# vuyraj/Data-Compression-Implementing-GPU-Driven-Huffman-Encoding-in-Java

Hardware: AMD Instinct MI355X
Metric: encode+decode GB/s (input bytes) (higher is better)
Workload: dtype u8

## Files before the change

data-compression-implementing-gpu-driven-huffman-encoding-in-java_amd/csrc/k1_histogram.hip:

```cpp
#include "dcz_internal.h"

namespace dcz {

#ifndef DCZ_K1_COPIES
#define DCZ_K1_COPIES 16
#endif
#ifndef DCZ_K1_NT
#define DCZ_K1_NT 1
#endif
#ifndef DCZ_K1_COPY_NT
#define DCZ_K1_COPY_NT 1
#endif
#ifndef DCZ_K1_COPY_LATE
#define DCZ_K1_COPY_LATE 1
#endif
#ifndef DCZ_K1_WAVES
#define DCZ_K1_WAVES 4
#endif
#ifndef DCZ_K1_RUNS
#define DCZ_K1_RUNS 1
#endif
constexpr int K1_WAVES = DCZ_K1_WAVES;
constexpr int K1_COPIES = DCZ_K1_COPIES;
constexpr int K1_CSHIFT = (K1_COPIES == 32) ? 5 : (K1_COPIES == 16) ? 4 : 3;
// ... 8 lines not shown
template <int K>
__device__ __forceinline__ void hist_add_byte(uint32_t hcol_addr, uint32_t d) {
    typedef __attribute__((address_space(3))) uint32_t lds_u32;
    uint32_t t, addr, b, val;
    asm("v_bfe_u32 %0, %1, %2, 7" : "=v"(t) : "v"(d), "n"(8 * K));
    asm("v_lshl_add_u32 %0, %1, %2, %3" : "=v"(addr) : "v"(t), "n"(K1_CSHIFT + 2), "v"(hcol_addr));
    asm("v_bfe_u32 %0, %1, %2, 1" : "=v"(b) : "v"(d), "n"(8 * K + 7));
    asm("v_mad_u32_u24 %0, %1, %2, 1" : "=v"(val) : "v"(b), "s"(0xFFFFu));
    __hip_atomic_fetch_add((lds_u32*)(uintptr_t)addr, val, __ATOMIC_RELAXED, __HIP_MEMORY_SCOPE_WAVEFRONT);
}

__device__ __forceinline__ void hist_add_dword(uint32_t* h, uint32_t col, uint32_t d) {
    const uint32_t hcol_addr = (uint32_t)(uintptr_t)((__attribute__((address_space(3))) uint32_t*)(h + col));
    hist_add_byte<0>(hcol_addr, d);
    hist_add_byte<1>(hcol_addr, d);
    hist_add_byte<2>(hcol_addr, d);
    hist_add_byte<3>(hcol_addr, d);
}

__device__ __forceinline__ void hist_add_vec(uint32_t* h, uint32_t col, const uint4& v) {
    hist_add_dword(h, col, v.x);
    hist_add_dword(h, col, v.y);
    hist_add_dword(h, col, v.z);
    hist_add_dword(h, col, v.w);
}

__device__ __forceinline__ bool unit_is_run(const uint4& v) {
    return v.x == v.y && v.x == v.z && v.x == v.w && v.x == __builtin_amdgcn_alignbit(v.x, v.x, 8);
}
__device__ __forceinline__ void hist_add_vec_runs(uint32_t* h, uint32_t col, const uint4& v) {
    if (unit_is_run(v)) {
        const uint32_t byte = v.x & 0xFFu;
        const uint32_t idx = ((byte & 127u) << K1_CSHIFT) + col;
        const uint32_t val = ((byte >> 7) * 0xFFFFu + 1u) << 4;
        __hip_atomic_fetch_add(&h[idx], val, __ATOMIC_RELAXED, __HIP_MEMORY_SCOPE_WAVEFRONT);
    } else {
        hist_add_vec(h, col, v);
    }
}

template <bool COPY>
__global__ __launch_bounds__(K1_WAVES * 64) void k1_histogram(const uint8_t* __restrict__ in, size_t n,
                                                               size_t block_bytes, uint32_t spb, uint64_t nseg,
                                                               uint16_t* __restrict__ seg_hist,
                                                               uint8_t* __restrict__ copy_out) {
    __shared__ __attribute__((aligned(16))) uint32_t lds[K1_WAVES][K1_DW];
    const int w = (int)(threadIdx.x >> 6);
    const int lane = lane_id();
    const uint64_t seg = (uint64_t)blockIdx.x * K1_WAVES + (uint64_t)w;
    if (seg >= nseg) return;
    uint32_t* h = lds[w];
    const uint32_t col = (uint32_t)lane & (uint32_t)(K1_COPIES - 1);

    {
        uint4* h4 = reinterpret_cast<uint4*>(h);
        const uint4 z = make_uint4(0, 0, 0, 0);
#pragma unroll
        for (int i = 0; i < K1_DW / 4 / 64; i++) h4[i * 64 + lane] = z;
    }
    wave_lds_fence();

    const uint64_t b = seg / spb, j = seg % spb;
    const uint64_t bstart = b * (uint64_t)block_bytes;
    const uint64_t bend = (bstart + block_bytes < n) ? bstart + block_bytes : (uint64_t)n;
    const uint64_t s0 = bstart + j * (uint64_t)SEG;
    uint32_t len = 0;
    if (s0 < bend) len = (uint32_t)((bend - s0 < SEG) ? bend - s0 : SEG);
    const uint8_t* p = in + s0;

    uint32_t nhead = (uint32_t)((16u - ((uintptr_t)p & 15u)) & 15u);
    if (nhead > len) nhead = len;
    if ((uint32_t)lane < nhead) {
        const uint8_t v = p[lane];
        hist_add(h, col, v);
        if constexpr (COPY) copy_out[s0 + lane] = v;
    }
    const uint4* pv = reinterpret_cast<const uint4*>(p + nhead);
    u32x4* const cv = COPY ? reinterpret_cast<u32x4*>(copy_out + s0 + nhead) : nullptr;
    auto store4 = [&](uint32_t base, const uint4& d0, const uint4& d1, const uint4& d2, const uint4& d3) {
        if constexpr (COPY) {
            const uint32_t i0 = base + (uint32_t)lane;
            const u32x4 a = {d0.x, d0.y, d0.z, d0.w}, b2 = {d1.x, d1.y, d1.z, d1.w};
            const u32x4 c = {d2.x, d2.y, d2.z, d2.w}, e = {d3.x, d3.y, d3.z, d3.w};
#if DCZ_K1_COPY_NT
            __builtin_nontemporal_store(a, cv + i0);
            __builtin_nontemporal_store(b2, cv + i0 + 64);
            __builtin_nontemporal_store(c, cv + i0 + 128);
            __builtin_nontemporal_store(e, cv + i0 + 192);
#else
            cv[i0] = a;
            cv[i0 + 64] = b2;
            cv[i0 + 128] = c;
            cv[i0 + 192] = e;
#endif
        }
    };
    const uint32_t nvec = (len - nhead) >> 4;

    auto load4 = [&](uint32_t base, uint4& d0, uint4& d1, uint4& d2, uint4& d3) {
        const uint32_t i0 = base + (uint32_t)lane;
#if DCZ_K1_NT
        const u32x4* pn = reinterpret_cast<const u32x4*>(pv);
        const u32x4 n0 = __builtin_nontemporal_load(pn + i0), n1 = __builtin_nontemporal_load(pn + i0 + 64);
        const u32x4 n2 = __builtin_nontemporal_load(pn + i0 + 128), n3 = __builtin_nontemporal_load(pn + i0 + 192);
        d0 = make_uint4(n0.x, n0.y, n0.z, n0.w);
        d1 = make_uint4(n1.x, n1.y, n1.z, n1.w);
        d2 = make_uint4(n2.x, n2.y, n2.z, n2.w);
        d3 = make_uint4(n3.x, n3.y, n3.z, n3.w);
#else
        d0 = pv[i0];
        d1 = pv[i0 + 64];
        d2 = pv[i0 + 128];
        d3 = pv[i0 + 192];
#endif
    };
    const uint32_t nfull = nvec & ~255u;
    uint4 c0, c1, c2, c3;
    if (nfull) load4(0, c0, c1, c2, c3);
    for (uint32_t base = 0; base < nfull; base += 256) {
        uint4 n0 = c0, n1 = c1, n2 = c2, n3 = c3;
        if (base + 256 < nfull) load4(base + 256, n0, n1, n2, n3);
#if !DCZ_K1_COPY_LATE
        store4(base, c0, c1, c2, c3);
#endif
        if (DCZ_K1_RUNS && __builtin_popcountll(__builtin_amdgcn_ballot_w64(unit_is_run(c0))) >= 32) {
            hist_add_vec_runs(h, col, c0);
            hist_add_vec_runs(h, col, c1);
            hist_add_vec_runs(h, col, c2);
            hist_add_vec_runs(h, col, c3);
        } else {
            hist_add_vec(h, col, c0);
            hist_add_vec(h, col, c1);
            hist_add_vec(h, col, c2);
            hist_add_vec(h, col, c3);
        }
#if DCZ_K1_COPY_LATE
        store4(base, c0, c1, c2, c3);
#endif
        c0 = n0;
        c1 = n1;
        c2 = n2;
        c3 = n3;
    }
    for (uint32_t i = nfull + (uint32_t)lane; i < nvec; i += 64) {
        const uint4 v = pv[i];
        hist_add_vec(h, col, v);
        if constexpr (COPY) {
            const u32x4 a = {v.x, v.y, v.z, v.w};
            __builtin_nontemporal_store(a, cv + i);
        }
    }
    {
        const uint32_t done = nhead + (nvec << 4);
        const uint32_t ntail = len - done;
        if ((uint32_t)lane < ntail) {
            const uint8_t v = p[done + lane];
            hist_add(h, col, v);
            if constexpr (COPY) copy_out[s0 + done + lane] = v;
        }
    }
    wave_lds_fence();

    uint32_t acc0 = 0, acc1 = 0;
    const uint4* r0 = reinterpret_cast<const uint4*>(h + (uint32_t)lane * (uint32_t)K1_COPIES);
    const uint4* r1 = reinterpret_cast<const uint4*>(h + ((uint32_t)lane + 64u) * (uint32_t)K1_COPIES);
    constexpr int NQ = K1_COPIES / 4;
#pragma unroll
    for (int t = 0; t < NQ; t++) {
        const int q = (t + (lane >> 1)) & (NQ - 1);
        const uint4 a = r0[q];
        const uint4 c = r1[q];
// ... 44 lines not shown
```

data-compression-implementing-gpu-driven-huffman-encoding-in-java_amd/csrc/k4_dfa.hip:

```cpp
#include <cstdlib>
#include <utility>

#include "dcz_internal.h"

namespace dcz {

#ifndef DCZ_DFA_W
#define DCZ_DFA_W 256
#endif
#ifndef DCZ_DFA_OC
#define DCZ_DFA_OC 16384
#endif
#ifndef DCZ_DFA_HOIST
#define DCZ_DFA_HOIST 1
#endif
#define DFA_RJ_DECL uint32_t rfresh_ = 0
#define DFA_RJ(rj, ALWAYS)                                                     \
    if constexpr ((j & 7) == 0 && ((ALWAYS) || (j >> 3) >= HOIST_DW)) {        \
        rfresh_ = R[j >> 3];                                                   \
        asm volatile("" : "+v"(rfresh_));                                      \
    }                                                                          \
    const uint32_t rj = ((ALWAYS) || (j >> 3) >= HOIST_DW) ? rfresh_ : R[j >> 3]
#ifndef DCZ_DFA_HOIST_DW_SPLIT
#define DCZ_DFA_HOIST_DW_SPLIT 3
#endif
#ifndef DCZ_DFA_HOIST_DW_REC
#define DCZ_DFA_HOIST_DW_REC 0
#endif
#ifndef DCZ_DFA_HOIST_DW_COUNT
#define DCZ_DFA_HOIST_DW_COUNT 8
#endif
#ifndef DCZ_DFA_HOIST_DW_1024
#define DCZ_DFA_HOIST_DW_1024 5
#endif
#ifndef DCZ_DFA_X_FROM
#define DCZ_DFA_X_FROM 16
#endif
#ifndef DCZ_DFA_KATTR
#define DCZ_DFA_KATTR
#endif
#ifndef DCZ_DFA_ALLWALK
#define DCZ_DFA_ALLWALK 0
#endif
#ifndef DCZ_DFA_X6_BIT0
#define DCZ_DFA_X6_BIT0 64
#endif
#ifndef DCZ_DFA_X_FROM_SPARSE
#define DCZ_DFA_X_FROM_SPARSE 48
#endif
#ifndef DCZ_DFA_SPARSE_OC
#define DCZ_DFA_SPARSE_OC 16384
#endif
#ifndef DCZ_DFA_ABL
#define DCZ_DFA_ABL 0
#endif
#ifndef DCZ_DFA_DBG
#define DCZ_DFA_DBG 0
#endif
#ifndef DCZ_DFA_X6
#define DCZ_DFA_X6 1
#endif
#ifndef DCZ_DFA_RECORD
#define DCZ_DFA_RECORD 1
#endif
#ifndef DCZ_DFA_MINWAVES
#define DCZ_DFA_MINWAVES 4
#endif
#define DFA_OC_DECODE (DCZ_DFA_RECORD ? -1 : DCZ_DFA_OC)
#ifndef DCZ_K4_EXACT_AFTER
#define DCZ_K4_EXACT_AFTER 12
#endif
#ifndef DCZ_K4_CLS2_A
#define DCZ_K4_CLS2_A 4
#endif
#ifndef DCZ_K4_CLS2_B
#define DCZ_K4_CLS2_B 9
#endif

constexpr uint32_t DFA_ERR = 255;

#ifndef DCZ_DFA_SLOT_SMALL
#define DCZ_DFA_SLOT_SMALL 88
#endif
#ifndef DCZ_DFA_REC_AVG
#define DCZ_DFA_REC_AVG 60
#endif
constexpr int dfa_slot(int W) { return W > 512 ? 136 : DCZ_DFA_SLOT_SMALL; }
#ifndef DCZ_DFA_PCAP
#define DCZ_DFA_PCAP 12
#endif
constexpr int DFA_PCAP = DCZ_DFA_PCAP;
template <int W, int OC, int PL = 0>
struct DfaLds {
    static constexpr int CAP = (OC < 0) ? (16 + dfa_slot(W) * W - 512) : (OC + 512);
    static constexpr int TILE_BYTES = PL ? (OC + 64) : (CAP + 640);
    __attribute__((aligned(16))) uint32_t T[256 * 16];
    union {
        __attribute__((aligned(16))) uint32_t tile[TILE_BYTES / 4];
        struct {
            uint32_t node_p[256];
            uint32_t first[34], cnt[34], offs[34], nint[34], base[34];
            uint8_t node_l[256];
            uint8_t symtab[256], len8[256];
        };
    };
    uint16_t plist[PL ? W * (PL + 1) + 128 : 2];
    uint8_t exits[W];
    uint32_t wsum[W / 64];
    uint32_t flag[3];
    uint32_t maxlen, nstates, err_idx, cend_vote, zsym;
    int bad_table;
};

template <int W, class LdsT>
__device__ __forceinline__ uint32_t dfa_block_scan(uint32_t v, LdsT& L, uint32_t& total) {
    const uint32_t inc = wave_inclusive_scan_u32(v);
    __syncthreads();
    if ((threadIdx.x & 63u) == 63u) L.wsum[threadIdx.x >> 6] = inc;
    __syncthreads();
    uint32_t base = 0, tot = 0;
#pragma unroll
    for (int w = 0; w < W / 64; w++) {
        const uint32_t sv = L.wsum[w];
        if (w < (int)(threadIdx.x >> 6)) base += sv;
        tot += sv;
    }
    total = tot;
    return base + inc - v;
}

template <int Q>
__device__ __forceinline__ uint4 dfa_shift(const uint4& a, const uint4& b, uint32_t r) {
    const uint32_t d[8] = {a.x, a.y, a.z, a.w, b.x, b.y, b.z, b.w};
    return make_uint4(__builtin_amdgcn_alignbyte(d[Q + 1], d[Q], r), __builtin_amdgcn_alignbyte(d[Q + 2], d[Q + 1], r),
                      __builtin_amdgcn_alignbyte(d[Q + 3], d[Q + 2], r), __builtin_amdgcn_alignbyte(d[Q + 4], d[Q + 3], r));
}

#if DCZ_DFA_DBG
__device__ unsigned long long dfa_dbg[8];
#endif
#if DCZ_K4_PROF
__device__ unsigned long long dfa_prof[12];
#define DFA_T(i)                                  \
    do {                                          \
        const unsigned long long t_ = clock64();  \
        pacc[i] += t_ - plast;                    \
        plast = t_;                               \
    } while (0)
#else
#define DFA_T(i) do { } while (0)
#endif

template <int W, int OC, int MODE, bool SPARSE>
__global__ __launch_bounds__(W, W > 512 ? 1 : DCZ_DFA_MINWAVES) DCZ_DFA_KATTR void k4_dfa(
    const uint8_t* __restrict__ comp, const unsigned long long* __restrict__ d_comp_off,
    const uint32_t* __restrict__ d_comp_size, const uint32_t* __restrict__ d_orig_size, const uint8_t* __restrict__ d_len,
    size_t out_stride, uint8_t* __restrict__ out, int32_t* __restrict__ d_status, long long* __restrict__ d_errpos,
    uint8_t* __restrict__ d_cls, const SplitDesc* __restrict__ sdp) {
    using LdsT = DfaLds<W, OC, SPARSE ? DFA_PCAP : 0>;
    constexpr bool SPLIT = MODE == 1, COUNT = MODE == 2;
    constexpr bool RECORD = OC < 0;
    static_assert(!RECORD || (!SPARSE && !COUNT), "only the decoding passes of the dense automaton record");
    constexpr int HOIST_DW = !DCZ_DFA_HOIST ? 0 : SPLIT ? DCZ_DFA_HOIST_DW_SPLIT : W > 512 ? DCZ_DFA_HOIST_DW_1024 : COUNT ? DCZ_DFA_HOIST_DW_COUNT : DCZ_DFA_HOIST_DW_REC;
    __shared__ LdsT L;
    typedef __attribute__((address_space(3))) const uint32_t lds_cu32;
    typedef __attribute__((address_space(3))) uint32_t lds_u32;
    uint32_t b = blockIdx.x, reg = 0;
    const int tid = (int)threadIdx.x;
#if DCZ_K4_PROF
    unsigned long long pacc[12] = {0, 0, 0, 0, 0, 0, 0, 0, 0, 0, 0, 0};
    unsigned long long plast = clock64();
#endif
    if constexpr (SPLIT) {
        if (!split_region_of(sdp, blockIdx.x, b, reg)) return;
        if (d_cls[b] != 2 || reg >= sdp->nreg[b]) return;
    } else if constexpr (COUNT) {
        if (!split_region_of(sdp, blockIdx.x, b, reg)) return;
        if (d_cls[b] != 0) return;
    } else {
        if (d_cls[b] != 0) return;
    }
    const uint32_t orig_blk = d_orig_size[b];
    const unsigned long long coff = d_comp_off[b];
    const uint32_t csize = d_comp_size[b];
    if constexpr (COUNT) {
        const unsigned long long S = sdp->region_bytes;
        const unsigned long long nreg = ((((uintptr_t)comp + (uintptr_t)coff) & 15u) + csize + S - 1) / S;
        if (nreg < 2 || reg >= nreg || nreg > sdp->rmax) return;
    }
    const uint32_t orig = SPLIT ? sdp->count[(uint64_t)b * sdp->rmax + reg] : COUNT ? 0xFFFFFFFFu : orig_blk;
    if (SPLIT && orig == 0u) return;
    {
        const bool long_codes = (unsigned long long)csize * 16ull >= (unsigned long long)orig_blk * 13ull;
        const bool medium = (unsigned long long)orig_blk * (unsigned long long)DCZ_K4_CLS2_A <=
                            (unsigned long long)csize * (unsigned long long)DCZ_K4_CLS2_B;
        if constexpr (SPARSE) {
            static_assert(!SPLIT, "regions of sparse blocks are decoded by k4_decode.hip");
            const bool sparse = (unsigned long long)csize * 80ull < (unsigned long long)orig_blk * 13ull;
            if (long_codes || medium || !sparse) return;
        } else {
            if (long_codes || !medium) return;
        }
    }

    if (tid < 34) L.cnt[tid] = 0;
    if (tid == 0) {
        L.bad_table = 0;
        L.err_idx = 0xFFFFFFFFu;
    }
    __syncthreads();
    for (int sy = tid; sy < 256; sy += W) {
        const uint32_t l = d_len[(uint64_t)b * 256u + sy];
        L.len8[sy] = (uint8_t)l;
        if (l > 32) L.bad_table = 1;
        else if (l > 0) atomicAdd(&L.cnt[l], 1u);
    }
    __syncthreads();
    if (tid == 0) {
        uint32_t c = 0, o = 0, mx = 0;
// ... 107 lines not shown
                    if (l > 32u) {
                        err = true;
                        break;
                    }
                    const uint32_t rel = p - L.first[l];
                    if (rel < L.cnt[l]) {
                        l = 0;
                        p = 0;
                    } else if (rel - L.cnt[l] >= L.nint[l]) {
                        err = true;
                    }
                }
                if (!err) next = L.base[l] + (p - L.first[l] - L.cnt[l]);
            }
            x6[idx] = (uint8_t)next;
        }
    }
    const uint32_t t_addr = (uint32_t)(uintptr_t)((__attribute__((address_space(3))) uint32_t*)(&L.T[0]));
    const uint32_t tile_addr = (uint32_t)(uintptr_t)((__attribute__((address_space(3))) uint32_t*)(&L.tile[0]));

    uint8_t* const oblk = out + (uint64_t)b * out_stride + (SPLIT ? sdp->off[(uint64_t)b * sdp->rmax + reg] : 0u);
    uint32_t hskip = SPLIT ? (uint32_t)(((uintptr_t)oblk) & 15u) : 0u;
    uint8_t* const obase = oblk - hskip;
    const bool out_aligned = (((uintptr_t)obase) & 15u) == 0u;
    const uintptr_t pay = (uintptr_t)comp + (uintptr_t)coff;
    const uint32_t skew = (uint32_t)(pay & 15u);
    const uint8_t* const vbase = reinterpret_cast<const uint8_t*>(pay - skew);
    const unsigned long long vlo = skew, vhi = (unsigned long long)skew + csize;

    uint32_t produced = 0, gpos = 0, ocarry = hskip;
    uint32_t entry0 = 0;
    unsigned long long wbyte = 0;
    uint32_t nwin = 0xFFFFFFFFu;
    bool preroll = false;
    if constexpr (SPLIT) {
        wbyte = (unsigned long long)reg * sdp->region_bytes;
        entry0 = sdp->entry[(uint64_t)b * sdp->rmax + reg];
    }
    if constexpr (COUNT) {
        const unsigned long long S = sdp->region_bytes;
        nwin = (uint32_t)(S / ((unsigned long long)W * 32ull));
        wbyte = (unsigned long long)reg * S;
        if (reg > 0) {
            wbyte -= (unsigned long long)W * 32ull;
            nwin++;
            preroll = true;
        }
    }
    int status = DCZ_OK;
    long long errpos = 0;
    constexpr uint32_t AMASK = SPARSE ? 0x3FC0u : 0xFFC0u;
    uint8_t* const ob = reinterpret_cast<uint8_t*>(L.tile);

    uint4 pre[3];
    auto prefetch = [&](unsigned long long wb) {
        const unsigned long long v0 = (wb + 32ull * (unsigned long long)tid + skew) & ~15ull;
#pragma unroll
        for (int c = 0; c < 3; c++) pre[c] = load_chunk16(vbase, v0 + 16ull * c, vlo, vhi);
    };
    const uint32_t sk2 = (skew + (uint32_t)(wbyte & 15ull)) & 15u;
    const uint32_t sq = sk2 >> 2, sr = sk2 & 3u;
    if (orig > 0 && wbyte < csize) prefetch(wbyte);
    const uint32_t slot_addr = tile_addr + 16u + (uint32_t)dfa_slot(W) * (uint32_t)tid;
    __syncthreads();
    const bool rec_block = RECORD && (dfa_slot(W) - 8 >= 128 || (unsigned long long)orig_blk * 32ull <=
                                                               (unsigned long long)csize * (unsigned long long)DCZ_DFA_REC_AVG);
    auto zero_tile = [&](uint32_t from16) {
        for (uint32_t i = from16 + (uint32_t)tid; i < (uint32_t)(sizeof(L.tile) / 16u); i += W)
            reinterpret_cast<uint4*>(L.tile)[i] = make_uint4(0u, 0u, 0u, 0u);
        __syncthreads();
    };
    if (!rec_block) zero_tile(0u);
    typedef __attribute__((address_space(3))) uint16_t lds_u16;
    typedef __attribute__((address_space(3))) uint8_t lds_u8;
    const uint32_t pl_addr = (uint32_t)(uintptr_t)((__attribute__((address_space(3))) uint16_t*)(&L.plist[0])) +
                             2u * (uint32_t)(DFA_PCAP + 1) * (uint32_t)tid;
    DFA_T(0);

    uint32_t rentry = 0, wexit = 0;
    unsigned long long rcount = 0;
    bool unusable = false;
    while (COUNT ? nwin != 0u : produced < orig) {
#if DCZ_K4_PROF
        pacc[8]++;
#endif
        uint32_t R[8];
        {
            uint4 lo, hi;
            switch (sq) {
                case 0: lo = dfa_shift<0>(pre[0], pre[1], sr); hi = dfa_shift<0>(pre[1], pre[2], sr); break;
                case 1: lo = dfa_shift<1>(pre[0], pre[1], sr); hi = dfa_shift<1>(pre[1], pre[2], sr); break;
                case 2: lo = dfa_shift<2>(pre[0], pre[1], sr); hi = dfa_shift<2>(pre[1], pre[2], sr); break;
                default: lo = dfa_shift<3>(pre[0], pre[1], sr); hi = dfa_shift<3>(pre[1], pre[2], sr); break;
            }
            R[0] = bswap32(lo.x);
            R[1] = bswap32(lo.y);
            R[2] = bswap32(lo.z);
            R[3] = bswap32(lo.w);
            R[4] = bswap32(hi.x);
            R[5] = bswap32(hi.y);
            R[6] = bswap32(hi.z);
            R[7] = bswap32(hi.w);
        }
        DFA_T(1);
        const bool exhausted = wbyte + (unsigned long long)W * 32ull >= csize;
        const bool beyond = wbyte + 32ull * (unsigned long long)tid >= csize;
        const bool more_payload = !exhausted;
        if (more_payload) prefetch(wbyte + (unsigned long long)W * 32ull);

        uint32_t g = (tid == 0) ? entry0 : 0u;
        uint32_t x = 0, nsym = 0, pc = 0;
        bool pover = false;
        bool need = !beyond;
        uint32_t round = (DCZ_DFA_ABL & 4) ? 1u : 0u;
        while (true) {
            if (DCZ_DFA_ALLWALK || __builtin_amdgcn_ballot_w64(need) != 0ull) {
                uint32_t e = g << 6, n = 0;
                if (round == 0u && small) {
                    constexpr int X6_BIT0 = DCZ_DFA_X6_BIT0, X6_STEPS = (256 - X6_BIT0) / 6;
                    static_assert(X6_BIT0 + 6 * X6_STEPS == 256, "the six-bit walk ends on the subsequence's last bit");
                    uint32_t rq[8], st6 = 0;
#pragma unroll
                    for (int k = X6_BIT0 >> 5; k < 8; k++) {
                        rq[k] = R[k];
                        asm volatile("" : "+v"(rq[k]));
                    }
                    auto stepX6 = [&](auto ic) __attribute__((always_inline)) {
                        constexpr int pbit = X6_BIT0 + 6 * decltype(ic)::value, k = pbit >> 5, off = pbit & 31;
                        uint32_t v;
                        if constexpr (off <= 26) v = (rq[k] >> (26 - off)) & 63u;
                        else v = __builtin_amdgcn_alignbit(rq[k], rq[k < 7 ? k + 1 : 7], 58 - off) & 63u;
                        st6 = (uint32_t)*(const lds_u8*)(uintptr_t)(t_addr + 8192u + ((st6 << 6) | v));
                    };
                    [&]<int... Is>(std::integer_sequence<int, Is...>) {
                        (stepX6(std::integral_constant<int, Is>{}), ...);
                    }(std::make_integer_sequence<int, X6_STEPS>{});
                    e = st6 << 6;
                } else if (round == 0u) {
                    constexpr int XF = SPARSE ? DCZ_DFA_X_FROM_SPARSE : DCZ_DFA_X_FROM;
                    if (XF > 0) e = 0;
                    DFA_RJ_DECL;
                    auto stepX = [&](auto jc) __attribute__((always_inline)) {
                        constexpr int j = decltype(jc)::value;
                        constexpr int sh = 26 - 4 * (j & 7);
                        DFA_RJ(rj, false);
                        const uint32_t nib4 = sh >= 0 ? ((rj >> (sh >= 0 ? sh : 0)) & 0x3Cu) : ((rj << 2) & 0x3Cu);
                        e = *(lds_cu32*)(uintptr_t)(t_addr + ((e & AMASK) | nib4));
                    };
                    [&]<int... Js>(std::integer_sequence<int, Js...>) {
                        (stepX(std::integral_constant<int, XF + Js>{}), ...);
                    }(std::make_integer_sequence<int, 64 - XF>{});
                } else if constexpr (SPARSE) {
                    uint32_t pa = pl_addr;
                    DFA_RJ_DECL;
                    auto stepP = [&](auto jc) __attribute__((always_inline)) {
                        constexpr int j = decltype(jc)::value;
                        constexpr int sh = 26 - 4 * (j & 7);
                        DFA_RJ(rj, false);
                        const uint32_t nib4 = sh >= 0 ? ((rj >> (sh >= 0 ? sh : 0)) & 0x3Cu) : ((rj << 2) & 0x3Cu);
                        e = *(lds_cu32*)(uintptr_t)(t_addr + ((e & AMASK) | nib4));
                        const uint32_t oth = e & 0x18u;
                        const uint32_t tp = n + ((e >> 14) & 3u);
                        *(lds_u16*)(uintptr_t)pa = (uint16_t)(tp | ((e >> 8) & 0xFF00u));
                        if (__builtin_amdgcn_ballot_w64(oth == 0x10u) != 0ull) {
                            if (oth == 0x10u) {
                                *(lds_u16*)(uintptr_t)pa = (uint16_t)(n | ((e >> 8) & 0xFF00u));
                                *(lds_u16*)(uintptr_t)(pa + 2u) = (uint16_t)(tp | ((e >> 16) & 0xFF00u));
                            }
                        }
                        pa += oth >> 2;
                        n += e & 7u;
                    };
                    [&]<int... Js>(std::integer_sequence<int, Js...>) {
                        (stepP(std::integral_constant<int, Js>{}), ...);
                    }(std::make_integer_sequence<int, 64>{});
                    if (need) pc = (pa - pl_addr) >> 1;
                } else if (RECORD && rec_block) {
                    uint32_t ab = slot_addr, k8 = 0, alo = 0;
#if DCZ_DFA_DBG
                    uint32_t chk = 0;
#endif
                    DFA_RJ_DECL;
                    auto stepR = [&](auto jc) __attribute__((always_inline)) {
                        constexpr int j = 2 * decltype(jc)::value;
                        constexpr int sh0 = 26 - 4 * (j & 7), sh1 = 26 - 4 * ((j + 1) & 7);
                        DFA_RJ(rj, false);
                        const uint32_t nib0 = (rj >> sh0) & 0x3Cu;
                        const uint32_t nib1 = sh1 >= 0 ? ((rj >> (sh1 >= 0 ? sh1 : 0)) & 0x3Cu) : ((rj << 2) & 0x3Cu);
                        const uint32_t e0 = *(lds_cu32*)(uintptr_t)(t_addr + ((e & AMASK) | nib0));
                        e = *(lds_cu32*)(uintptr_t)(t_addr + ((e0 & AMASK) | nib1));
                        const uint32_t c0 = e0 & 0x18u;
                        const uint32_t w = ((e >> 16) << c0) | (e0 >> 16);
                        const unsigned long long v = (unsigned long long)w << k8;
#if DCZ_DFA_DBG
                        chk = __builtin_amdgcn_sad_u8(w, 0u, chk);
#endif
                        alo |= (uint32_t)v;
                        *(lds_u32*)(uintptr_t)ab = alo;
                        k8 += c0 + (e & 0x18u);
                        const bool full = k8 >= 32u;
                        alo = full ? (uint32_t)(v >> 32) : alo;
                        ab += full ? 4u : 0u;
                        k8 &= 31u;
                    };
                    [&]<int... Js>(std::integer_sequence<int, Js...>) {
                        (stepR(std::integral_constant<int, Js>{}), ...);
                    }(std::make_integer_sequence<int, 32>{});
                    *(lds_u32*)(uintptr_t)ab = alo;
                    n = (ab - slot_addr) + (k8 >> 3);
#if DCZ_DFA_DBG
                    *(lds_u32*)(uintptr_t)(slot_addr + (uint32_t)dfa_slot(W) - 4u) = (n & 0xFFu) | (chk << 8);
#endif
                } else {
                    DFA_RJ_DECL;
                    auto stepA = [&](auto jc) __attribute__((always_inline)) {
                        constexpr int j = decltype(jc)::value;
                        constexpr int sh = 26 - 4 * (j & 7);
                        DFA_RJ(rj, RECORD || SPARSE);
                        const uint32_t nib4 = sh >= 0 ? ((rj >> (sh >= 0 ? sh : 0)) & 0x3Cu) : ((rj << 2) & 0x3Cu);
                        e = *(lds_cu32*)(uintptr_t)(t_addr + ((e & AMASK) | nib4));
                        n += e & (SPARSE ? 7u : 3u);
                    };
                    [&]<int... Js>(std::integer_sequence<int, Js...>) {
                        (stepA(std::integral_constant<int, Js>{}), ...);
                    }(std::make_integer_sequence<int, 64>{});
                }
                if (need) {
                    x = (e >> 6) & 0xFFu;
                    nsym = n;
                    if constexpr (SPARSE) pover |= pc > (uint32_t)DFA_PCAP;
                    else if constexpr (RECORD) pover |= n > (uint32_t)dfa_slot(W) - 8u;
                }
            }
            DFA_T(2);
#if DCZ_K4_PROF
            pacc[9]++;
#endif
            L.exits[tid] = (uint8_t)x;
            if (tid == 0) L.flag[(round + 1u) % 3u] = 0;
            __syncthreads();
            DFA_T(3);
            if (round > 1u && L.flag[round % 3u] == 0u) break;
            if (DCZ_DFA_ABL & 16) break;
            const uint32_t ng = (tid == 0) ? entry0 : (uint32_t)L.exits[tid - 1];
            need = ((ng != g) || round == 0u) && !beyond;
            g = ng;
            if (__builtin_amdgcn_ballot_w64(need) != 0ull && (tid & 63) == 0) L.flag[(round + 1u) % 3u] = 1;
            round++;
            if constexpr (MODE == 0 && !SPARSE) {
                if (round == (uint32_t)DCZ_K4_EXACT_AFTER) {
                    if (tid == 0) d_cls[b] = 1;
                    return;
                }
            }
            if constexpr (COUNT) {
                if (round == (uint32_t)DCZ_K4_EXACT_AFTER) {
                    if (tid == 0) sdp->exit[(uint64_t)b * sdp->rmax + reg] = 0xFFFFFFFFu;
                    return;
                }
            }
        }

        const bool bad = !beyond && x == errst;
        uint32_t tw = 0;
        constexpr uint32_t SLOT_SYMS = RECORD ? (uint32_t)dfa_slot(W) - 8u : 0u;
// ... 295 lines not shown
                        alo = ahi;
                        ahi = 0;
                        k8 -= 32u;
                        ab += 4u;
                    }
                };
                [&]<int... Js>(std::integer_sequence<int, Js...>) {
                    (stepB(std::integral_constant<int, Js>{}), ...);
                }(std::make_integer_sequence<int, 32>{});
            }
            __syncthreads();
            if (k8 != 0u)
                __hip_atomic_fetch_or((lds_u32*)(uintptr_t)ab, alo, __ATOMIC_RELAXED, __HIP_MEMORY_SCOPE_WORKGROUP);
            DFA_T(5);
#if DCZ_K4_PROF
            pacc[10]++;
#endif
            __syncthreads();
            DFA_T(6);
            const uint32_t total = ocarry + cc;
            const bool last = !more && cend == lim;
            const uint32_t full = last ? total : (total & ~15u);
            uint8_t* const dst = obase + gpos;
            const uint32_t nunits = (full + 15u) >> 4;
            for (uint32_t u = (uint32_t)tid; u < nunits; u += W) {
                const uint32_t lo = u << 4;
                const uint32_t* src = &L.tile[lo >> 2];
                if (out_aligned && lo + 16u <= full && lo >= hskip) {
                    *reinterpret_cast<uint4*>(dst + lo) = make_uint4(src[0], src[1], src[2], src[3]);
                } else {
                    for (uint32_t i = lo > hskip ? lo : hskip; i < lo + 16u && i < full; i++) dst[i] = ob[i];
                }
                *reinterpret_cast<uint4*>(&L.tile[lo >> 2]) = make_uint4(0u, 0u, 0u, 0u);
            }
            const uint32_t tail = total - full;
            uint8_t tv = 0;
            if ((uint32_t)tid < tail) tv = ob[full + tid];
            __syncthreads();
            if (full > 0u) {
                if (tid < 4) L.tile[(full >> 2) + (uint32_t)tid] = 0u;
                if ((uint32_t)tid < tail) ob[tid] = tv;
            }
            gpos += full;
            ocarry = tail;
            if (full > 0u) hskip = 0;
            cbase = cend;
            DFA_T(7);
            if (cbase < lim) __syncthreads();
        }
        }
        }
        produced += lim;
        entry0 = next_entry;
        wbyte += (unsigned long long)W * 32ull;
        if (exhausted && produced < orig) {
            __syncthreads();
            if ((uint32_t)tid < ocarry && (uint32_t)tid >= hskip) obase[gpos + tid] = (uint8_t)(ob[tid] ^ (SPARSE ? L.zsym : 0u));
            const uint8_t z = L.zsym;
            uint32_t fs = z;
            if (tid == 0) {
                uint32_t st = wexit;
                while (st != 0u) {
                    const uint32_t e = L.T[st * 16u];
                    if ((e & (SPARSE ? 7u : 3u)) != 0u) {
                        fs = (e >> 16) & 0xFFu;
                        break;
                    }
                    st = (e >> 6) & 0xFFu;
                    if (st == errst) {
                        status = DCZ_E_BADSTREAM;
                        errpos = (long long)produced;
                        break;
                    }
                }
            }
            for (uint32_t i = produced + (uint32_t)tid; i < orig; i += W) oblk[i] = (i == produced) ? (uint8_t)fs : z;
            break;
        }
        __syncthreads();
    }

    if constexpr (COUNT) {
        if (tid == 0) {
            const uint64_t i = (uint64_t)b * sdp->rmax + reg;
            const bool bad = unusable || wexit == errst || rentry == errst;
            sdp->entry[i] = rentry;
            sdp->count[i] = (uint32_t)(rcount > 0xFFFFFFFFull ? 0xFFFFFFFFull : rcount);
            sdp->exit[i] = bad ? 0xFFFFFFFFu : wexit;
        }
        return;
    }
    if (tid == 0 && (!SPLIT || status != DCZ_OK)) {
        d_status[b] = status;
        if (d_errpos) d_errpos[b] = errpos + (SPLIT ? (long long)sdp->off[(uint64_t)b * sdp->rmax + reg] : 0ll);
    }
#if DCZ_K4_PROF
    if (tid == 0)
        for (int i = 0; i < 12; i++) atomicAdd(&dfa_prof[i], pacc[i]);
#endif
}

void launch_count_dfa(const uint8_t* d_comp, const uint64_t* d_comp_off, const uint32_t* d_comp_size,
                      const uint32_t* d_orig_size, const uint8_t* d_len, uint8_t* d_cls, const SplitDesc* d_sd, hipStream_t s) {
    hipLaunchKernelGGL((k4_dfa<DCZ_DFA_W, 0, 2, false>), dim3(SPLIT_GRID), dim3(DCZ_DFA_W), 0, s, d_comp,
                       reinterpret_cast<const unsigned long long*>(d_comp_off), d_comp_size, d_orig_size, d_len, (size_t)0,
                       (uint8_t*)nullptr, (int32_t*)nullptr, (long long*)nullptr, d_cls, d_sd);
// ... 55 lines not shown
```

data-compression-implementing-gpu-driven-huffman-encoding-in-java_amd/csrc/k4_fixed.hip:

```cpp
#include "dcz_internal.h"

namespace dcz {

#ifndef DCZ_FX_TILE
#define DCZ_FX_TILE 8192
#endif
constexpr uint32_t FX_TILE = DCZ_FX_TILE;
#ifndef DCZ_FX_T
#define DCZ_FX_T 512
#endif
constexpr int FX_T = DCZ_FX_T;
constexpr int FX_UPT = (int)(FX_TILE / 16u / (uint32_t)FX_T);
static_assert(FX_T >= 256 && FX_UPT * FX_T * 16 == (int)FX_TILE, "tile = threads x units x 16 bytes");

__global__ __launch_bounds__(256) void k4_classify(const uint8_t* __restrict__ d_len,
                                                   const unsigned long long* __restrict__ d_comp_off,
                                                   const uint32_t* __restrict__ d_comp_size,
                                                   const uint32_t* __restrict__ d_orig_size, unsigned long long comp_bytes,
                                                   unsigned long long out_stride, uint32_t K, uint8_t* __restrict__ cls,
                                                   int32_t* __restrict__ d_status, long long* __restrict__ d_errpos,
                                                   uint32_t* __restrict__ hint, uint32_t* __restrict__ hint_done,
                                                   uint32_t epoch) {
    const uint32_t b = blockIdx.x * 256u + threadIdx.x;
    if (b >= K) return;
// ... 28 lines not shown
    cls[b] = c;
    if ((c & 0xF0u) == 0x10u && hint) *hint = epoch;
}

template <int Q>
__device__ __forceinline__ uint4 shift_units(const uint4& a, const uint4& b, uint32_t r) {
    const uint32_t d[8] = {a.x, a.y, a.z, a.w, b.x, b.y, b.z, b.w};
    return make_uint4(__builtin_amdgcn_alignbyte(d[Q + 1], d[Q], r), __builtin_amdgcn_alignbyte(d[Q + 2], d[Q + 1], r),
                      __builtin_amdgcn_alignbyte(d[Q + 3], d[Q + 2], r), __builtin_amdgcn_alignbyte(d[Q + 4], d[Q + 3], r));
}

__device__ __forceinline__ void store_unit(uint8_t* dst, const uint4& v, uint32_t nvalid, bool aligned) {
    if (aligned && nvalid >= 16u) {
        *reinterpret_cast<uint4*>(dst) = v;
    } else {
        const uint32_t w[4] = {v.x, v.y, v.z, v.w};
#pragma unroll
        for (int i = 0; i < 16; i++)
            if ((uint32_t)i < nvalid) dst[i] = (uint8_t)(w[i >> 2] >> (8 * (i & 3)));
    }
}

template <int L>
__device__ __forceinline__ uint4 extract16(const uint32_t (&bw)[5], const uint8_t* symtab) {
    uint32_t o[4] = {0, 0, 0, 0};
#pragma unroll
    for (int j = 0; j < 16; j++) {
        constexpr uint32_t mask = (1u << L) - 1u;
        const int bit = j * L, idx = bit >> 5, s = bit & 31;
        uint32_t v;
        if (s + L <= 32) v = (bw[idx] >> (32 - s - L)) & mask;
        else v = (uint32_t)((((unsigned long long)bw[idx] << 32) | bw[idx + 1]) >> (64 - s - L)) & mask;
        o[j >> 2] |= (uint32_t)symtab[v] << (8 * (j & 3));
    }
    return make_uint4(o[0], o[1], o[2], o[3]);
}

struct FxLds {
    __attribute__((aligned(16))) uint32_t stage[(FX_TILE / 8 * 7 + 64) / 4];
    uint8_t symtab[256];
    uint32_t wcnt[FX_T / 64];
};

__device__ __forceinline__ void fixed_item(FxLds& S, uint32_t b, uint32_t tile, const uint8_t* __restrict__ comp,
                                           const unsigned long long* __restrict__ d_comp_off,
                                           const uint32_t* __restrict__ d_comp_size,
                                           const uint32_t* __restrict__ d_orig_size, const uint8_t* __restrict__ d_len,
                                           unsigned long long out_stride, uint8_t* __restrict__ out,
                                           const uint8_t* __restrict__ cls) {
    uint32_t* const stage = S.stage;
    uint8_t* const symtab = S.symtab;
    uint32_t* const wcnt = S.wcnt;
    const uint32_t c = cls[b];
    if ((c & 0xF0u) != 0x10u) return;
    const uint32_t L = c & 15u;
    const int tid = (int)threadIdx.x;
    const uint32_t orig = d_orig_size[b];
    const unsigned long long t0 = (unsigned long long)tile * FX_TILE;
    if (t0 >= orig) return;
    const uint32_t nout = (orig - t0 < FX_TILE) ? (uint32_t)(orig - t0) : FX_TILE;
    const uintptr_t pay = (uintptr_t)comp + (uintptr_t)d_comp_off[b];
    const uint32_t skew = (uint32_t)(pay & 15u);
    const uint8_t* const vbase = reinterpret_cast<const uint8_t*>(pay - skew);
    const unsigned long long vlo = skew, vhi = (unsigned long long)skew + d_comp_size[b];
    uint8_t* const dst0 = out + (unsigned long long)b * out_stride + t0;
    const bool dst_al = (((uintptr_t)dst0) & 15u) == 0u;
    if (L == 8u) {
        if (skew == 0u && dst_al && nout == FX_TILE && t0 + FX_TILE <= vhi) {
            const u32x4* s4 = reinterpret_cast<const u32x4*>(vbase + t0) + tid;
            u32x4* d4 = reinterpret_cast<u32x4*>(dst0) + tid;
            u32x4 v[FX_UPT];
#pragma unroll
            for (int k = 0; k < FX_UPT; k++) v[k] = __builtin_nontemporal_load(s4 + FX_T * k);
#pragma unroll
            for (int k = 0; k < FX_UPT; k++) __builtin_nontemporal_store(v[k], d4 + FX_T * k);
            return;
        }
        uint4 v[FX_UPT];
        const uint32_t q = skew >> 2, r = skew & 3u;
#pragma unroll
        for (int k = 0; k < FX_UPT; k++) {
            const uint32_t o = ((uint32_t)tid + (uint32_t)FX_T * k) * 16u;
            v[k] = make_uint4(0, 0, 0, 0);
            if (o < nout) {
                const uint4 a = load_chunk16(vbase, t0 + o, vlo, vhi);
                if (skew == 0u) {
                    v[k] = a;
                } else {
                    const uint4 e = load_chunk16(vbase, t0 + o + 16u, vlo, vhi);
                    v[k] = (q == 0u) ? shift_units<0>(a, e, r) : (q == 1u) ? shift_units<1>(a, e, r)
                           : (q == 2u) ? shift_units<2>(a, e, r) : shift_units<3>(a, e, r);
                }
            }
        }
#pragma unroll
        for (int k = 0; k < FX_UPT; k++) {
            const uint32_t o = ((uint32_t)tid + (uint32_t)FX_T * k) * 16u;
            if (o < nout) store_unit(dst0 + o, v[k], nout - o, dst_al);
        }
        return;
    }
    {
        const bool present = tid < 256 && d_len[(uint64_t)b * 256u + (tid & 255)] != 0;
        const unsigned long long m = __builtin_amdgcn_ballot_w64(present);
        if (tid < 256 && (tid & 63) == 0) wcnt[tid >> 6] = (uint32_t)__builtin_popcountll(m);
        __syncthreads();
        uint32_t rank = (uint32_t)__builtin_popcountll(m & ((1ull << (tid & 63)) - 1ull));
        for (int w = 0; w < ((tid & 255) >> 6); w++) rank += wcnt[w];
        if (present) symtab[rank] = (uint8_t)tid;
    }
    const unsigned long long vin = (t0 >> 3) * L;
    const uint32_t nin = (nout * L + 7u) >> 3;
    const uint32_t nchunks = (skew + nin + 15u) >> 4;
    for (uint32_t ch = (uint32_t)tid; ch < nchunks; ch += FX_T)
        reinterpret_cast<uint4*>(stage)[ch] = load_chunk16(vbase, vin + 16ull * ch, vlo, vhi);
    __syncthreads();
#pragma unroll 1
// ... 111 lines not shown
```

Measured before the change: 1413.

## Overlap next-window DFA entry walk with current decode, defer histogram zeroing

The DFA decode kernel now computes the next window's starting state (the six-bit or nibble walk) while the current window's record/sparse walk is running, interleaving the independent LDS lookups to hide latency. The next payload is unpacked mid-walk, and the separate round-0 walk is skipped on later windows. The histogram kernel issues its first global loads before zeroing LDS and adding head bytes, and the fixed-length decoder hoists its metadata loads above the early return. This raises register pressure and code size and adds tail-masking logic for the pipelined unpack.

```diff
diff --git a/data-compression-implementing-gpu-driven-huffman-encoding-in-java_amd/csrc/k1_histogram.hip b/data-compression-implementing-gpu-driven-huffman-encoding-in-java_amd/csrc/k1_histogram.hip
--- a/data-compression-implementing-gpu-driven-huffman-encoding-in-java_amd/csrc/k1_histogram.hip
+++ b/data-compression-implementing-gpu-driven-huffman-encoding-in-java_amd/csrc/k1_histogram.hip
@@ -84,14 +84,6 @@
     uint32_t* h = lds[w];
     const uint32_t col = (uint32_t)lane & (uint32_t)(K1_COPIES - 1);
 
-    {
-        uint4* h4 = reinterpret_cast<uint4*>(h);
-        const uint4 z = make_uint4(0, 0, 0, 0);
-#pragma unroll
-        for (int i = 0; i < K1_DW / 4 / 64; i++) h4[i * 64 + lane] = z;
-    }
-    wave_lds_fence();
-
     const uint64_t b = seg / spb, j = seg % spb;
     const uint64_t bstart = b * (uint64_t)block_bytes;
     const uint64_t bend = (bstart + block_bytes < n) ? bstart + block_bytes : (uint64_t)n;
@@ -102,10 +94,10 @@
 
     uint32_t nhead = (uint32_t)((16u - ((uintptr_t)p & 15u)) & 15u);
     if (nhead > len) nhead = len;
+    uint8_t headv = 0;
     if ((uint32_t)lane < nhead) {
-        const uint8_t v = p[lane];
-        hist_add(h, col, v);
-        if constexpr (COPY) copy_out[s0 + lane] = v;
+        headv = p[lane];
+        if constexpr (COPY) copy_out[s0 + lane] = headv;
     }
     const uint4* pv = reinterpret_cast<const uint4*>(p + nhead);
     u32x4* const cv = COPY ? reinterpret_cast<u32x4*>(copy_out + s0 + nhead) : nullptr;
@@ -149,6 +141,14 @@
     const uint32_t nfull = nvec & ~255u;
     uint4 c0, c1, c2, c3;
     if (nfull) load4(0, c0, c1, c2, c3);
+    {
+        uint4* h4 = reinterpret_cast<uint4*>(h);
+        const uint4 z = make_uint4(0, 0, 0, 0);
+#pragma unroll
+        for (int i = 0; i < K1_DW / 4 / 64; i++) h4[i * 64 + lane] = z;
+    }
+    wave_lds_fence();
+    if ((uint32_t)lane < nhead) hist_add(h, col, headv);
     for (uint32_t base = 0; base < nfull; base += 256) {
         uint4 n0 = c0, n1 = c1, n2 = c2, n3 = c3;
         if (base + 256 < nfull) load4(base + 256, n0, n1, n2, n3);
diff --git a/data-compression-implementing-gpu-driven-huffman-encoding-in-java_amd/csrc/k4_dfa.hip b/data-compression-implementing-gpu-driven-huffman-encoding-in-java_amd/csrc/k4_dfa.hip
--- a/data-compression-implementing-gpu-driven-huffman-encoding-in-java_amd/csrc/k4_dfa.hip
+++ b/data-compression-implementing-gpu-driven-huffman-encoding-in-java_amd/csrc/k4_dfa.hip
@@ -48,6 +48,12 @@
 #ifndef DCZ_DFA_X_FROM_SPARSE
 #define DCZ_DFA_X_FROM_SPARSE 48
 #endif
+#ifndef DCZ_DFA_PIPE
+#define DCZ_DFA_PIPE 1
+#endif
+#ifndef DCZ_DFA_PIPE_1024
+#define DCZ_DFA_PIPE_1024 0
+#endif
 #ifndef DCZ_DFA_SPARSE_OC
 #define DCZ_DFA_SPARSE_OC 16384
 #endif
@@ -78,6 +84,15 @@
 #endif
 
 constexpr uint32_t DFA_ERR = 255;
+
+#ifndef DCZ_DFA_PIPE_LAG
+#define DCZ_DFA_PIPE_LAG 8
+#endif
+constexpr int dfa_x6_at(int i, int steps) {
+    constexpr int lag = DCZ_DFA_PIPE_LAG;
+    const int a = i < lag ? 0 : i < 2 * lag ? 2 * (i - lag) : i;
+    return a < steps ? a : steps;
+}
 
 #ifndef DCZ_DFA_SLOT_SMALL
 #define DCZ_DFA_SLOT_SMALL 88
@@ -165,6 +180,8 @@
     __shared__ LdsT L;
     typedef __attribute__((address_space(3))) const uint32_t lds_cu32;
     typedef __attribute__((address_space(3))) uint32_t lds_u32;
+    typedef __attribute__((address_space(3))) uint16_t lds_u16;
+    typedef __attribute__((address_space(3))) uint8_t lds_u8;
     uint32_t b = blockIdx.x, reg = 0;
     const int tid = (int)threadIdx.x;
 #if DCZ_K4_PROF
@@ -378,14 +395,78 @@
     constexpr uint32_t AMASK = SPARSE ? 0x3FC0u : 0xFFC0u;
     uint8_t* const ob = reinterpret_cast<uint8_t*>(L.tile);
 
+    typedef uint32_t u32x4 __attribute__((ext_vector_type(4)));
+    typedef __attribute__((address_space(1))) const u32x4 glb_cu4;
     uint4 pre[3];
     auto prefetch = [&](unsigned long long wb) {
         const unsigned long long v0 = (wb + 32ull * (unsigned long long)tid + skew) & ~15ull;
 #pragma unroll
-        for (int c = 0; c < 3; c++) pre[c] = load_chunk16(vbase, v0 + 16ull * c, vlo, vhi);
+        for (int c = 0; c < 3; c++) {
+            const unsigned long long vb = v0 + 16ull * c;
+            pre[c] = make_uint4(0u, 0u, 0u, 0u);
+            if (vb + 16ull > vlo && vb < vhi) {
+                const u32x4 t = *(glb_cu4*)(uintptr_t)(vbase + vb);
+                pre[c] = make_uint4(t.x, t.y, t.z, t.w);
+            }
+        }
     };
     const uint32_t sk2 = (skew + (uint32_t)(wbyte & 15ull)) & 15u;
     const uint32_t sq = sk2 >> 2, sr = sk2 & 3u;
+    auto unpack = [&](uint32_t (&d)[8], unsigned long long wb, uint32_t sr) __attribute__((always_inline)) {
+        uint4 lo, hi;
+        switch (sq) {
+            case 0: lo = dfa_shift<0>(pre[0], pre[1], sr); hi = dfa_shift<0>(pre[1], pre[2], sr); break;
+            case 1: lo = dfa_shift<1>(pre[0], pre[1], sr); hi = dfa_shift<1>(pre[1], pre[2], sr); break;
+            case 2: lo = dfa_shift<2>(pre[0], pre[1], sr); hi = dfa_shift<2>(pre[1], pre[2], sr); break;
+            default: lo = dfa_shift<3>(pre[0], pre[1], sr); hi = dfa_shift<3>(pre[1], pre[2], sr); break;
+        }
+        d[0] = bswap32(lo.x);
+        d[1] = bswap32(lo.y);
+        d[2] = bswap32(lo.z);
+        d[3] = bswap32(lo.w);
+        d[4] = bswap32(hi.x);
+        d[5] = bswap32(hi.y);
+        d[6] = bswap32(hi.z);
+        d[7] = bswap32(hi.w);
+        if (wb + (unsigned long long)W * 32ull > csize) {
+            const unsigned long long pb = wb + 32ull * (unsigned long long)tid;
+            const uint32_t nv = pb >= csize ? 0u : csize - pb >= 32ull ? 32u : (uint32_t)(csize - pb);
+#pragma unroll
+            for (int k = 0; k < 8; k++) {
+                const uint32_t vk = nv > 4u * k ? (nv - 4u * k < 4u ? nv - 4u * k : 4u) : 0u;
+                d[k] &= (uint32_t)(0xFFFFFFFF00000000ull >> (8u * vk));
+            }
+        }
+    };
+    auto unpack_next = [&](uint32_t (&d)[8], int from, unsigned long long wb) __attribute__((always_inline)) {
+        uint32_t srq = sr;
+        asm volatile("" : "+s"(srq));
+        unpack(d, wb, srq);
+#pragma unroll
+        for (int k = 0; k < 8; k++)
+            if (k >= from) asm volatile("" : "+v"(d[k]));
+    };
+    constexpr int X6_BIT0 = DCZ_DFA_X6_BIT0, X6_STEPS = (256 - X6_BIT0) / 6;
+    static_assert(X6_BIT0 + 6 * X6_STEPS == 256, "the six-bit walk ends on the subsequence's last bit");
+    auto x6step = [&](const uint32_t (&q)[8], uint32_t& st, auto ic) __attribute__((always_inline)) {
+        constexpr int pbit = X6_BIT0 + 6 * decltype(ic)::value, k = pbit >> 5, off = pbit & 31;
+        uint32_t v;
+        if constexpr (off <= 26) v = (q[k] >> (26 - off)) & 63u;
+        else v = __builtin_amdgcn_alignbit(q[k], q[k < 7 ? k + 1 : 7], 58 - off) & 63u;
+        st = (uint32_t)*(const lds_u8*)(uintptr_t)(t_addr + 8192u + ((st << 6) | v));
+    };
+    constexpr int XF = SPARSE ? DCZ_DFA_X_FROM_SPARSE : DCZ_DFA_X_FROM;
+    auto xnstep = [&](const uint32_t (&q)[8], uint32_t& e, auto jc) __attribute__((always_inline)) {
+        constexpr int j = XF + decltype(jc)::value;
+        constexpr int sh = 26 - 4 * (j & 7);
+        const uint32_t qj = q[j >> 3];
+        const uint32_t nib4 = sh >= 0 ? ((qj >> (sh >= 0 ? sh : 0)) & 0x3Cu) : ((qj << 2) & 0x3Cu);
+        e = *(lds_cu32*)(uintptr_t)(t_addr + ((e & AMASK) | nib4));
+    };
+    constexpr bool PIPE = DCZ_DFA_PIPE && MODE == 0 && !(DCZ_DFA_ABL & 20) &&
+                          (SPARSE ? W <= 512 : RECORD && (W <= 512 || DCZ_DFA_PIPE_1024));
+    static_assert(X6_STEPS <= 32 && 64 - XF <= 64 && 2 * DCZ_DFA_PIPE_LAG <= 32, "PIPE: the walks ride along with 32 pair-steps");
+    uint32_t xg = 0, xg_next = 0;
     if (orig > 0 && wbyte < csize) prefetch(wbyte);
     const uint32_t slot_addr = tile_addr + 16u + (uint32_t)dfa_slot(W) * (uint32_t)tid;
     __syncthreads();
@@ -397,8 +478,6 @@
         __syncthreads();
     };
     if (!rec_block) zero_tile(0u);
-    typedef __attribute__((address_space(3))) uint16_t lds_u16;
-    typedef __attribute__((address_space(3))) uint8_t lds_u8;
     const uint32_t pl_addr = (uint32_t)(uintptr_t)((__attribute__((address_space(3))) uint16_t*)(&L.plist[0])) +
                              2u * (uint32_t)(DFA_PCAP + 1) * (uint32_t)tid;
     DFA_T(0);
@@ -411,28 +490,15 @@
         pacc[8]++;
 #endif
         uint32_t R[8];
-        {
-            uint4 lo, hi;
-            switch (sq) {
-                case 0: lo = dfa_shift<0>(pre[0], pre[1], sr); hi = dfa_shift<0>(pre[1], pre[2], sr); break;
-                case 1: lo = dfa_shift<1>(pre[0], pre[1], sr); hi = dfa_shift<1>(pre[1], pre[2], sr); break;
-                case 2: lo = dfa_shift<2>(pre[0], pre[1], sr); hi = dfa_shift<2>(pre[1], pre[2], sr); break;
-                default: lo = dfa_shift<3>(pre[0], pre[1], sr); hi = dfa_shift<3>(pre[1], pre[2], sr); break;
-            }
-            R[0] = bswap32(lo.x);
-            R[1] = bswap32(lo.y);
-            R[2] = bswap32(lo.z);
-            R[3] = bswap32(lo.w);
-            R[4] = bswap32(hi.x);
-            R[5] = bswap32(hi.y);
-            R[6] = bswap32(hi.z);
-            R[7] = bswap32(hi.w);
-        }
+        unpack(R, wbyte, sr);
         DFA_T(1);
         const bool exhausted = wbyte + (unsigned long long)W * 32ull >= csize;
         const bool beyond = wbyte + 32ull * (unsigned long long)tid >= csize;
         const bool more_payload = !exhausted;
         if (more_payload) prefetch(wbyte + (unsigned long long)W * 32ull);
+        const bool pipe_blk = PIPE && (SPARSE || (rec_block && small));
+        const bool pipe_now = pipe_blk && more_payload;
+        const bool piped = pipe_blk && wbyte != 0ull;
 
         uint32_t g = (tid == 0) ? entry0 : 0u;
         uint32_t x = 0, nsym = 0, pc = 0;
@@ -442,28 +508,20 @@
         while (true) {
             if (DCZ_DFA_ALLWALK || __builtin_amdgcn_ballot_w64(need) != 0ull) {
                 uint32_t e = g << 6, n = 0;
-                if (round == 0u && small) {
-                    constexpr int X6_BIT0 = DCZ_DFA_X6_BIT0, X6_STEPS = (256 - X6_BIT0) / 6;
-                    static_assert(X6_BIT0 + 6 * X6_STEPS == 256, "the six-bit walk ends on the subsequence's last bit");
+                if (PIPE && round == 0u && piped) {
+                    e = xg << 6;
+                } else if (round == 0u && small) {
                     uint32_t rq[8], st6 = 0;
 #pragma unroll
                     for (int k = X6_BIT0 >> 5; k < 8; k++) {
                         rq[k] = R[k];
                         asm volatile("" : "+v"(rq[k]));
                     }
-                    auto stepX6 = [&](auto ic) __attribute__((always_inline)) {
-                        constexpr int pbit = X6_BIT0 + 6 * decltype(ic)::value, k = pbit >> 5, off = pbit & 31;
-                        uint32_t v;
-                        if constexpr (off <= 26) v = (rq[k] >> (26 - off)) & 63u;
-                        else v = __builtin_amdgcn_alignbit(rq[k], rq[k < 7 ? k + 1 : 7], 58 - off) & 63u;
-                        st6 = (uint32_t)*(const lds_u8*)(uintptr_t)(t_addr + 8192u + ((st6 << 6) | v));
-                    };
                     [&]<int... Is>(std::integer_sequence<int, Is...>) {
-                        (stepX6(std::integral_constant<int, Is>{}), ...);
+                        (x6step(rq, st6, std::integral_constant<int, Is>{}), ...);
                     }(std::make_integer_sequence<int, X6_STEPS>{});
                     e = st6 << 6;
                 } else if (round == 0u) {
-                    constexpr int XF = SPARSE ? DCZ_DFA_X_FROM_SPARSE : DCZ_DFA_X_FROM;
                     if (XF > 0) e = 0;
                     DFA_RJ_DECL;
                     auto stepX = [&](auto jc) __attribute__((always_inline)) {
@@ -477,6 +535,9 @@
                         (stepX(std::integral_constant<int, XF + Js>{}), ...);
                     }(std::make_integer_sequence<int, 64 - XF>{});
                 } else if constexpr (SPARSE) {
+                    auto walkP = [&](auto pc_) __attribute__((always_inline)) {
+                    constexpr bool P = decltype(pc_)::value;
+                    uint32_t nq[8], en = 0;
                     uint32_t pa = pl_addr;
                     DFA_RJ_DECL;
                     auto stepP = [&](auto jc) __attribute__((always_inline)) {
@@ -484,7 +545,9 @@
                         constexpr int sh = 26 - 4 * (j & 7);
                         DFA_RJ(rj, false);
                         const uint32_t nib4 = sh >= 0 ? ((rj >> (sh >= 0 ? sh : 0)) & 0x3Cu) : ((rj << 2) & 0x3Cu);
+                        if constexpr (P && j == XF) unpack_next(nq, XF >> 3, wbyte + (unsigned long long)W * 32ull);
                         e = *(lds_cu32*)(uintptr_t)(t_addr + ((e & AMASK) | nib4));
+                        if constexpr (P && j >= XF) xnstep(nq, en, std::integral_constant<int, j - XF>{});
                         const uint32_t oth = e & 0x18u;
                         const uint32_t tp = n + ((e >> 14) & 3u);
                         *(lds_u16*)(uintptr_t)pa = (uint16_t)(tp | ((e >> 8) & 0xFF00u));
@@ -501,20 +564,36 @@
                         (stepP(std::integral_constant<int, Js>{}), ...);
                     }(std::make_integer_sequence<int, 64>{});
                     if (need) pc = (pa - pl_addr) >> 1;
+                    if constexpr (P) xg_next = (en >> 6) & 0xFFu;
+                    };
+                    if constexpr (PIPE) {
+                        if (pipe_now && round == 1u) walkP(std::true_type{});
+                        else walkP(std::false_type{});
+                    } else {
+                        walkP(std::false_type{});
+                    }
                 } else if (RECORD && rec_block) {
+                    auto walkR = [&](auto pc_) __attribute__((always_inline)) {
+                    constexpr bool P = decltype(pc_)::value;
+                    uint32_t nq[8], stn = 0;
                     uint32_t ab = slot_addr, k8 = 0, alo = 0;
 #if DCZ_DFA_DBG
                     uint32_t chk = 0;
 #endif
                     DFA_RJ_DECL;
                     auto stepR = [&](auto jc) __attribute__((always_inline)) {
-                        constexpr int j = 2 * decltype(jc)::value;
+                        constexpr int i = decltype(jc)::value, j = 2 * i;
                         constexpr int sh0 = 26 - 4 * (j & 7), sh1 = 26 - 4 * ((j + 1) & 7);
+                        constexpr int xa = dfa_x6_at(i, X6_STEPS), xb = dfa_x6_at(i + 1, X6_STEPS);
                         DFA_RJ(rj, false);
+                        if constexpr (P && i == DCZ_DFA_PIPE_LAG)
+                            unpack_next(nq, X6_BIT0 >> 5, wbyte + (unsigned long long)W * 32ull);
                         const uint32_t nib0 = (rj >> sh0) & 0x3Cu;
                         const uint32_t nib1 = sh1 >= 0 ? ((rj >> (sh1 >= 0 ? sh1 : 0)) & 0x3Cu) : ((rj << 2) & 0x3Cu);
                         const uint32_t e0 = *(lds_cu32*)(uintptr_t)(t_addr + ((e & AMASK) | nib0));
+                        if constexpr (P && xa < xb) x6step(nq, stn, std::integral_constant<int, xa>{});
                         e = *(lds_cu32*)(uintptr_t)(t_addr + ((e0 & AMASK) | nib1));
+                        if constexpr (P && xa + 1 < xb) x6step(nq, stn, std::integral_constant<int, xa + 1>{});
                         const uint32_t c0 = e0 & 0x18u;
                         const uint32_t w = ((e >> 16) << c0) | (e0 >> 16);
                         const unsigned long long v = (unsigned long long)w << k8;
@@ -537,6 +616,14 @@
 #if DCZ_DFA_DBG
                     *(lds_u32*)(uintptr_t)(slot_addr + (uint32_t)dfa_slot(W) - 4u) = (n & 0xFFu) | (chk << 8);
 #endif
+                    if constexpr (P) xg_next = stn;
+                    };
+                    if constexpr (PIPE) {
+                        if (pipe_now && round == 1u) walkR(std::true_type{});
+                        else walkR(std::false_type{});
+                    } else {
+                        walkR(std::false_type{});
+                    }
                 } else {
                     DFA_RJ_DECL;
                     auto stepA = [&](auto jc) __attribute__((always_inline)) {
@@ -938,6 +1025,7 @@
         }
         produced += lim;
         entry0 = next_entry;
+        xg = xg_next;
         wbyte += (unsigned long long)W * 32ull;
         if (exhausted && produced < orig) {
             __syncthreads();
diff --git a/data-compression-implementing-gpu-driven-huffman-encoding-in-java_amd/csrc/k4_fixed.hip b/data-compression-implementing-gpu-driven-huffman-encoding-in-java_amd/csrc/k4_fixed.hip
--- a/data-compression-implementing-gpu-driven-huffman-encoding-in-java_amd/csrc/k4_fixed.hip
+++ b/data-compression-implementing-gpu-driven-huffman-encoding-in-java_amd/csrc/k4_fixed.hip
@@ -104,17 +104,20 @@
     uint8_t* const symtab = S.symtab;
     uint32_t* const wcnt = S.wcnt;
     const uint32_t c = cls[b];
+    const uint32_t orig = d_orig_size[b];
+    const unsigned long long coff = d_comp_off[b];
+    const uint32_t csize = d_comp_size[b];
+    asm volatile("" ::"s"(orig), "s"(coff), "s"(csize));
     if ((c & 0xF0u) != 0x10u) return;
     const uint32_t L = c & 15u;
     const int tid = (int)threadIdx.x;
-    const uint32_t orig = d_orig_size[b];
     const unsigned long long t0 = (unsigned long long)tile * FX_TILE;
     if (t0 >= orig) return;
     const uint32_t nout = (orig - t0 < FX_TILE) ? (uint32_t)(orig - t0) : FX_TILE;
-    const uintptr_t pay = (uintptr_t)comp + (uintptr_t)d_comp_off[b];
+    const uintptr_t pay = (uintptr_t)comp + (uintptr_t)coff;
     const uint32_t skew = (uint32_t)(pay & 15u);
     const uint8_t* const vbase = reinterpret_cast<const uint8_t*>(pay - skew);
-    const unsigned long long vlo = skew, vhi = (unsigned long long)skew + d_comp_size[b];
+    const unsigned long long vlo = skew, vhi = (unsigned long long)skew + csize;
     uint8_t* const dst0 = out + (unsigned long long)b * out_stride + t0;
     const bool dst_al = (((uintptr_t)dst0) & 15u) == 0u;
     if (L == 8u) {
```

Result: faster. 1440, median of 6 (+1.9%).
